# damesek/hnsw-clj

Hardware: AMD Instinct MI355X
Metric: QPS @ recall@10>=0.98 (31k x 768, k=10); IVF scan achieved HBM GB/s vs roofline (higher is better)
Workload: dtype f32; 1 GPU; hnsw search-knn (ultra_fast.clj:346-374 = graph.clj:297-320), 31,173 x 768 f32 (clustered, java.util.Random seed 42; queries: the same generator, seed 43), k=10, M=16 ef_construction=200, index built on the device by the heuristic builder, batched HIP traversal kernel; builder=heuristic, ef_search=640, parallelism=replicas x1 (index replicated, queries sharded, no collective)

## Files before the change

hnsw-clj_amd/csrc/dense.hip:

```cpp
#include "engine.hpp"
#include "dense_kernels.hpp"
#include "wave_kernels.hpp"

namespace hg {

template <int N, int R, bool L>
static HnswKernelFn wave_dense_kernel(const HnswLaunchPlan &p) {
    return p.vis_global ? &hnsw_wave_kernel<N, R, L, true, false, true> : &hnsw_wave_kernel<N, R, L, false, false, true>;
}

HnswKernelFn hnsw_wave_dense_kernel_for(const HnswLaunchPlan &p, const HnswArgs &a) {
    const bool l2 = a.metric == METRIC_L2;
    if (p.nch == 3 && p.dense_rows == 4) return l2 ? wave_dense_kernel<3, 4, true>(p) : wave_dense_kernel<3, 4, false>(p);
#define PICK(N, R, RF) return l2 ? wave_dense_kernel<N, RF, true>(p) : wave_dense_kernel<N, RF, false>(p)
    HG_HNSW_ROWS(p.nch, 2, PICK);
#undef PICK
}

size_t hnsw_dense_code_bytes(int nch, int32_t nq) {
    return (sizeof(uint32_t) * 2 * kWave * nch * static_cast<size_t>(nq) + 255) & ~static_cast<size_t>(255);
}

int64_t hnsw_dense_ld(int64_t n) { return (n + kDenseTR - 1) / kDenseTR * kDenseTR; }

int launch_hnsw_dense(const hnswgpu_index *idx, const float *d_Q, int64_t qld, int32_t nq, void *codes, float *lb, int64_t lb_ld,
                      hipStream_t st) {
    QueryCodeArgs c;
    c.Q = d_Q;
    c.qld = qld;
    c.dim = idx->dim;
    c.nq = nq;
    c.qcode = static_cast<uint32_t *>(codes);
    c.qscal = reinterpret_cast<QueryScal *>(static_cast<char *>(codes) + hnsw_dense_code_bytes(idx->nch, nq));
    const int blocks = (nq + kNWave - 1) / kNWave;
#define CALL(N, R, L) hipLaunchKernelGGL((hnsw_query_code_kernel<N>), dim3(blocks), dim3(kWG), 0, st, c)
    HG_DISPATCH(idx->nch, false, CALL);
#undef CALL
    HG_HIP(hipGetLastError());
    DenseArgs d;
    d.qcode = c.qcode;
    d.qscal = c.qscal;
    d.qrows = idx->d_qrows;
    d.qmeta = idx->d_qmeta;
    d.lb = lb;
    d.lb_ld = lb_ld;
    d.n = idx->n;
    d.nq = nq;
    d.kbytes = 4 * kWave * idx->nch;
    d.metric = idx->metric;
    d.nqt = (nq + kDenseTQ - 1) / kDenseTQ;
    d.nrt = static_cast<int32_t>((idx->n + kDenseTR - 1) / kDenseTR);
    d.rp = std::max(1, std::min(kDensePanel, d.nrt / 8));
    d.nsp = (d.nrt + d.rp - 1) / d.rp;
    const int64_t grid = 8LL * ((d.nsp + 7) / 8) * d.nqt * d.rp;
    HG_REQUIRE(grid < (1LL << 31), HNSWGPU_ELIMIT, "too many tiles for one bounds launch");
    hipLaunchKernelGGL(hnsw_dense_bounds_kernel, dim3(static_cast<unsigned>(grid)), dim3(kWG), 0, st, d);
    HG_HIP(hipGetLastError());
    return 0;
}

}
```

hnsw-clj_amd/csrc/dense_kernels.hpp:

```cpp
#pragma once
#include "kernels.hpp"

namespace hg {

typedef int dense_v4i __attribute__((ext_vector_type(4)));
typedef int dense_v16i __attribute__((ext_vector_type(16)));

constexpr int kDenseTQ = 128;
constexpr int kDenseTR = 128;
constexpr int kDenseKS = 128;
constexpr int kDensePanel = 8;

struct QueryCodeArgs {
    const float *Q;
    int64_t qld;
    int32_t dim;
    int32_t nq;
    uint32_t *qcode;
    QueryScal *qscal;
};

template <int NCH>
__global__ __launch_bounds__(kWG) void hnsw_query_code_kernel(QueryCodeArgs a) {
    const int lane = threadIdx.x & (kWave - 1);
    const int qi = blockIdx.x * kNWave + (threadIdx.x >> 6);
    if (qi >= a.nq) return;
    float4 q[NCH];
    load_query<NCH>(q, a.Q + static_cast<int64_t>(qi) * a.qld, a.dim, lane);
    Query16<NCH> qc;
    encode_query16<NCH>(q, qc);
    uint32_t *hi = a.qcode + (static_cast<int64_t>(2 * qi) * kWave + lane) * NCH, *lo = hi + kWave * NCH;
#pragma unroll
    for (int c = 0; c < NCH; c++) {
        hi[c] = qc.hi[c];
        lo[c] = qc.lo[c];
    }
    if (lane == 0) a.qscal[qi] = qc.sc;
}

struct DenseArgs {
    const uint32_t *qcode;
    const QueryScal *qscal;
    const uint32_t *qrows;
    const float4 *qmeta;
    float *lb;
    int64_t lb_ld;
    int64_t n;
    int32_t nq;
    int32_t kbytes;
    int32_t metric;
    int32_t nqt, nrt;
    int32_t rp;
    int32_t nsp;
};

__device__ __forceinline__ int dense_lds_off(int row, int ks) { return row * kDenseKS + ((ks ^ ((row >> 1) & 7)) << 4); }

__global__ __launch_bounds__(kWG, 2) void hnsw_dense_bounds_kernel(DenseArgs a) {
    __shared__ __align__(16) unsigned char s_a[2 * kDenseTQ * kDenseKS];
    __shared__ __align__(16) unsigned char s_b[kDenseTR * kDenseKS];
    __shared__ QueryScal s_scal[kDenseTQ];
    const int tid = threadIdx.x, lane = tid & (kWave - 1), wv = tid >> 6;
    const int l31 = lane & 31, half = lane >> 5;
    const int xcd = blockIdx.x & 7, j = blockIdx.x >> 3;
    const int per = a.nqt * a.rp;
    const int sp = (j / per) * 8 + xcd, rem = j % per;
    const int qt = rem / a.rp, rt = sp * a.rp + rem % a.rp;
    if (sp >= a.nsp || rt >= a.nrt) return;
    const int q0 = qt * kDenseTQ;
    const int64_t r0 = static_cast<int64_t>(rt) * kDenseTR;
    const int64_t K = a.kbytes;

    if (tid < kDenseTQ) s_scal[tid] = a.qscal[q0 + tid < a.nq ? q0 + tid : a.nq - 1];
    const int ks = tid & 7, rr = tid >> 3;
    const unsigned char *const pa = reinterpret_cast<const unsigned char *>(a.qcode) + ks * 16;
    const unsigned char *const pb = reinterpret_cast<const unsigned char *>(a.qrows) + ks * 16;
    const int64_t a_last = 2LL * a.nq - 1, b_last = a.n - 1;
    dense_v4i va[8], vb[4];
#define HG_DENSE_FETCH(k0)                                                                       \
    do {                                                                                         \
        _Pragma("unroll") for (int i = 0; i < 8; i++) {                                          \
            const int64_t ar = static_cast<int64_t>(2 * q0) + rr + 32 * i;                       \
            va[i] = *reinterpret_cast<const dense_v4i *>(pa + (ar < a_last ? ar : a_last) * K + (k0)); \
        }                                                                                        \
        _Pragma("unroll") for (int i = 0; i < 4; i++) {                                          \
            const int64_t br = r0 + rr + 32 * i;                                                 \
            vb[i] = *reinterpret_cast<const dense_v4i *>(pb + (br < b_last ? br : b_last) * K + (k0)); \
        }                                                                                        \
    } while (0)
    dense_v16i acc[4][2];
#pragma unroll
    for (int sa = 0; sa < 4; sa++)
#pragma unroll
        for (int sb = 0; sb < 2; sb++)
#pragma unroll
            for (int g = 0; g < 16; g++) acc[sa][sb][g] = 0;
    const int arow = (wv >> 1) * 128 + l31, brow = (wv & 1) * 64 + l31;
    HG_DENSE_FETCH(0);
    for (int k0 = 0; k0 < a.kbytes; k0 += kDenseKS) {
#pragma unroll
        for (int i = 0; i < 8; i++) *reinterpret_cast<dense_v4i *>(s_a + dense_lds_off(rr + 32 * i, ks)) = va[i];
#pragma unroll
        for (int i = 0; i < 4; i++) *reinterpret_cast<dense_v4i *>(s_b + dense_lds_off(rr + 32 * i, ks)) = vb[i];
        __syncthreads();
        if (k0 + kDenseKS < a.kbytes) HG_DENSE_FETCH(k0 + kDenseKS);
#pragma unroll
        for (int u = 0; u < kDenseKS / 32; u++) {
            dense_v4i fa[4], fb[2];
#pragma unroll
            for (int sb = 0; sb < 2; sb++) fb[sb] = *reinterpret_cast<const dense_v4i *>(s_b + dense_lds_off(brow + 32 * sb, 2 * u + half));
#pragma unroll
            for (int sa = 0; sa < 4; sa++) fa[sa] = *reinterpret_cast<const dense_v4i *>(s_a + dense_lds_off(arow + 32 * sa, 2 * u + half));
#pragma unroll
            for (int sa = 0; sa < 4; sa++)
#pragma unroll
                for (int sb = 0; sb < 2; sb++) acc[sa][sb] = __builtin_amdgcn_mfma_i32_32x32x32_i8(fa[sa], fb[sb], acc[sa][sb], 0, 0, 0);
        }
        __syncthreads();
    }
#undef HG_DENSE_FETCH
#pragma unroll
    for (int sb = 0; sb < 2; sb++) {
        const int64_t row = r0 + (wv & 1) * 64 + 32 * sb + l31;
        const float4 meta = a.qmeta[row < a.n ? row : a.n - 1];
#pragma unroll
        for (int sa = 0; sa < 4; sa++) {
#pragma unroll
            for (int g = 0; g < 8; g++) {
                const int ql = (wv >> 1) * 64 + 16 * sa + 4 * (g >> 1) + 2 * half + (g & 1);
                const int tot = static_cast<int>(static_cast<unsigned>(acc[sa][sb][2 * g]) * 256u + static_cast<unsigned>(acc[sa][sb][2 * g + 1]));
                const float lb = code_lower_bound(a.metric, tot, s_scal[ql], meta, meta.w);
                if (q0 + ql < a.nq && row < a.n) a.lb[static_cast<int64_t>(q0 + ql) * a.lb_ld + row] = lb;
            }
        }
    }
}

}
```

hnsw-clj_amd/csrc/hnsw.hip:

```cpp
#include <math.h>
#include <stdlib.h>
#include <string.h>

#include <algorithm>
#include <chrono>
#include <condition_variable>
#include <functional>
#include <mutex>
#include <thread>
#include <vector>

#include "build_kernels.hpp"
#include "engine.hpp"
#include "hnsw_remove_kernels.hpp"
#include "hnsw_update_kernels.hpp"
#include "ivf_update_ids.hpp"
#include "lsh_remove_ids.hpp"
#include "javarandom.hpp"
#include "order_kernels.hpp"
#include "parts_kernels.hpp"
#include "solo_kernels.hpp"

namespace hg {

constexpr size_t kMaxLds = 160 * 1024;

static size_t hnsw_lds_bytes(int cap, int nwords, int nw) {
    return sizeof(uint2) * cap + sizeof(int32_t) * 3 * kMaxDeg + sizeof(int32_t) * 16 + sizeof(int32_t) * nw * kWave +
           sizeof(uint2) * kPfRing + sizeof(uint32_t) * nwords + sizeof(uint16_t) * cap + 16;
}

static size_t wave_lds_bytes(int cap, int nwords) {
    return sizeof(uint2) * cap + sizeof(uint2) * kWave + 2 * sizeof(int32_t) * kMaxDeg + sizeof(uint32_t) * nwords + 16;
}

constexpr int64_t kLdsVisitedMaxRows = 262144;
static_assert(kLdsVisitedMaxRows <= (1 << 18), "solo_tag holds 18 bits of a node id");
static bool hnsw_vis_global(int64_t n, int64_t vis_global_env) { return vis_global_env != 0 || n > kLdsVisitedMaxRows; }

constexpr int kPfMaxQueries = 128;
static_assert(kPfMaxQueries == kSoloMaxQueries, "one bound for both kinds of small launch");
constexpr int kSoloMinEf = 96;
constexpr int kOrderMinQueries = 10000;

static void hnsw_calibration_absorb(hnswgpu_index *idx) {
    if (idx->hnsw_cal_state != 1 || !idx->ev_hnsw_cal || hipEventQuery(idx->ev_hnsw_cal) != hipSuccess) return;
    const double f32_rows = static_cast<double>(idx->hnsw_cal_host[0]), nb = static_cast<double>(idx->hnsw_cal_host[1]);
    idx->hnsw_cal_frac = nb > 0 ? f32_rows / nb : 0.0;
    const double keep = static_cast<double>(tune(HNSWGPU_TUNE_HNSW_CALIBRATE_PCT, 65)) / 100.0;
    idx->hnsw_rej_off = nb > 0 && idx->hnsw_cal_frac > keep;
    idx->hnsw_cal_state = 2;
}

template <int N, int R, bool L>
static HnswKernelFn search_kernel(const HnswLaunchPlan &p) {
    if (p.kernel == HnswKernel::SearchHelpers) return &hnsw_search_kernel<N, R, L, 4, false, true>;
    if (p.vis_global) return p.nw == 1 ? &hnsw_search_kernel<N, R, L, 1, true> : (p.nw == 2 ? &hnsw_search_kernel<N, R, L, 2, true> : &hnsw_search_kernel<N, R, L, 4, true>);
    return p.nw == 1 ? &hnsw_search_kernel<N, R, L, 1, false> : (p.nw == 2 ? &hnsw_search_kernel<N, R, L, 2, false> : &hnsw_search_kernel<N, R, L, 4, false>);
}

static HnswKernelFn hnsw_search_kernel_for(const HnswLaunchPlan &p, const HnswArgs &a) {
    const bool l2 = a.metric == METRIC_L2;
#define PICK(N, R, RF) HG_HNSW_ROWS_IN_FLIGHT(search_kernel, N, R, RF)
    HG_HNSW_ROWS(p.nch, 2, PICK);
#undef PICK
}

static int hnsw_launch_plan(const hnswgpu_index *idx, const HnswArgs &a, const HnswLaunchPlan *first, HnswLaunchPlan &p,
                            bool plain_search = false) {
    memset(&p, 0, sizeof(p));
    const bool build = a.q_rows != nullptr, repeat = a.q_index != nullptr;
    const bool parts = a.items != nullptr;
    const int64_t vis_rows = parts ? idx->max_part : a.n;
    p.nch = idx->nch;
    p.rejection = a.qrows && (idx->rejection_mode == 2 || (idx->rejection_mode == 1 && a.nq >= 2 * idx->cus && idx->dim >= 128));
    if (p.rejection && idx->rejection_mode == 1 && !build && !repeat && tune(HNSWGPU_TUNE_HNSW_CALIBRATE, 1) != 0) {
        if (idx->hnsw_cal_state == 2 && idx->hnsw_rej_off) p.rejection = false;
        p.calibrate = idx->hnsw_cal_state == 0 && !(idx->prof && idx->d_rej_stats);
    }
    if (repeat) {
        p.kernel = HnswKernel::Search;
        p.vis_global = first->vis_global;
        p.nw = 4;
        p.grid = std::min(a.nq, 256);
    } else {
        const int64_t nw_raw = tune(HNSWGPU_TUNE_HNSW_NW, 0);
        const int nw_env = (nw_raw == 1 || nw_raw == 2 || nw_raw == 4) ? static_cast<int>(nw_raw) : 0;
        p.vis_global = hnsw_vis_global(vis_rows, tune(HNSWGPU_TUNE_VIS_GLOBAL, 0));
        const int64_t pf_env = tune(HNSWGPU_TUNE_PREFETCH, kTuneUnset);
        const int helper_groups = pf_env == kTuneUnset ? 4 : static_cast<int>(std::max<int64_t>(0, std::min<int64_t>(16, pf_env)));
        const int solo_groups = pf_env == kTuneUnset ? 8 : static_cast<int>(std::max<int64_t>(0, std::min<int64_t>(31, pf_env)));
        const bool small = helper_groups > 0 && !p.vis_global && !build && !parts && a.nq <= kPfMaxQueries && nw_env == 0 &&
                           a.n < (1LL << 31) && a.M0 <= kMaxDeg;
        const int64_t solo_mode = tune(HNSWGPU_TUNE_SOLO, 1);
        const bool solo = small && solo_groups > 0 && (solo_mode >= 2 || (solo_mode == 1 && a.ef >= kSoloMinEf));
        const int64_t hints_env = tune(HNSWGPU_TUNE_PF_HINTS, kTuneUnset);
        const auto hints = [hints_env](int dflt) {
            return static_cast<int32_t>(std::max<int64_t>(1, std::min<int64_t>(32, hints_env == kTuneUnset ? dflt : hints_env)));
        };
        int nw = nw_env > 0 ? nw_env : (a.nq > 1536 ? 1 : (a.nq > 768 ? 2 : 4));
        if (nw_env == 0 && p.rejection && p.nch <= 3) nw = a.nq > 2048 ? 1 : (a.nq > 1024 ? 2 : 4);
        const int nwords = p.vis_global ? 0 : a.nwords;
        const int64_t wave_mode = tune(HNSWGPU_TUNE_HNSW_WAVE, 1);
        const bool wave = wave_mode != 0 && !small && nw_env == 0 && wave_lds_bytes(a.cap, nwords) <= kMaxLds && a.M0 <= kMaxDeg &&
                          (wave_mode >= 2 || nw == 1 || a.ef >= 640);
        if (nw_env == 0 && !wave)
            while (nw < 4 && static_cast<int64_t>(kMaxLds / hnsw_lds_bytes(a.cap, nwords, nw)) * nw < 13) nw *= 2;
        p.grid = a.nq;
        if (solo) {
            p.kernel = HnswKernel::Solo;
            p.rejection = false;
            p.pf_groups = std::max(1, std::min(solo_groups, idx->cus / std::max(a.nq, 1) - 1));
            p.pf_hints = hints(a.ef < 256 ? 8 : 16);
            p.solo_chase = tune(HNSWGPU_TUNE_SOLO_CHASE, 1) != 0 ? 1 : 0;
            p.grid = 8 * ((a.nq + 7) / 8) * (1 + p.pf_groups);
            int log2s = static_cast<int>(tune(HNSWGPU_TUNE_SOLO_SLOTS, 0));
            if (log2s <= 0) {
                const int64_t want = std::min<int64_t>(a.n, 32LL * a.ef);
                log2s = 11;
                while ((1LL << log2s) < want && log2s < 18) log2s++;
                while (log2s > 11 && (static_cast<int64_t>(a.nq) << log2s) * a.M0 * 8 > (512LL << 20)) log2s--;
            }
            p.solo_log2s = std::max(8, std::min(log2s, 18));
            const size_t S = static_cast<size_t>(1) << p.solo_log2s;
            p.mail_bytes = (sizeof(uint32_t) * kSoloMailWords * kSoloMaxQueries + 255) & ~static_cast<size_t>(255);
            p.table_bytes = (sizeof(uint32_t) * S * a.nq + 255) & ~static_cast<size_t>(255);
            p.rec_bytes = sizeof(unsigned long long) * S * a.M0 * a.nq;
        } else if (small) {
            p.kernel = HnswKernel::SearchHelpers;
            nw = 4;
            p.pf_groups = std::max(1, std::min(helper_groups, idx->cus / std::max(a.nq, 1) - 1));
            p.pf_hints = hints(4);
            p.grid = 8 * ((a.nq + 7) / 8) * (1 + p.pf_groups);
            p.mail_bytes = sizeof(uint32_t) * kPfMailWords * kPfMaxQueries;
            p.table_bytes = sizeof(unsigned long long) * kPfMaxQueries * kPfRing * kMaxDeg;
            p.pf_eval = tune(HNSWGPU_TUNE_PF_EVAL, 1) != 0;
            if (p.pf_eval) p.rejection = false;
        } else {
            p.kernel = wave ? HnswKernel::Wave : HnswKernel::Search;
        }
        p.region = p.mail_bytes + p.table_bytes + p.rec_bytes;
        p.nw = nw;
        const int64_t order_mode = tune(HNSWGPU_TUNE_HNSW_ORDER, 1);
        p.ordered = p.kernel == HnswKernel::Wave && !build && !parts && idx->d_qrows && idx->d_qmeta &&
                    (order_mode >= 2 || (order_mode == 1 && a.nq >= kOrderMinQueries));
        if (p.ordered) p.grid = 8 * ((a.nq + 7) / 8);
        p.lb_ld = hnsw_dense_ld(a.n);
        const bool dense_rule = a.nq >= 8 * idx->cus && 6.5 * a.ef >= 0.06 * static_cast<double>(a.n);
        p.dense = plain_search && p.kernel == HnswKernel::Wave && p.rejection && !build && !parts && idx->dense_mode != 0 &&
                  static_cast<double>(a.nq) * static_cast<double>(p.lb_ld) * sizeof(float) <= static_cast<double>(idx->dense_budget) &&
                  (idx->dense_mode >= 2 || dense_rule);
        constexpr size_t kDenseRows4Lds = 7680;
        if (p.dense && p.nch == 3)
            p.dense_rows = idx->dense_rows_mode != 0 ? idx->dense_rows_mode : (wave_lds_bytes(a.cap, nwords) > kDenseRows4Lds ? 4 : 2);
    }
    p.nwords = p.vis_global ? 0 : a.nwords;
    if (p.vis_global) {
        const int64_t budget = 16LL << 30;
        int64_t max_wg = budget / (4 * std::max<int64_t>(a.n, 1));
        max_wg = std::min<int64_t>(std::max<int64_t>(max_wg, 256), 256 * 12);
        const int64_t slots = p.ordered ? 8 * ((static_cast<int64_t>(a.nq) + 7) / 8) : a.nq;
        p.grid = static_cast<int>(std::min<int64_t>(slots, max_wg));
        if (p.ordered) p.grid = std::max(8, p.grid & ~7);
        p.gens = (slots + p.grid - 1) / p.grid * (a.max_level + 1);
    }
    p.block = p.kernel == HnswKernel::Solo ? kWG : (p.kernel == HnswKernel::Wave ? kWave : p.nw * kWave);
    p.lds = p.kernel == HnswKernel::Solo   ? solo_lds_bytes(a.cap, p.nwords)
            : p.kernel == HnswKernel::Wave ? wave_lds_bytes(a.cap, p.nwords)
                                           : hnsw_lds_bytes(a.cap, p.nwords, p.nw);
    HG_REQUIRE(p.lds <= kMaxLds, HNSWGPU_ELIMIT, "HNSW search state (%zu B: ef=%d, n=%lld) exceeds the 160 KiB LDS of a CU", p.lds,
               a.ef, (long long)a.n);
    p.calibrate = p.calibrate && p.rejection;
    if (!build && !repeat) {
        const size_t fixed = hnsw_lds_bytes(0, p.nwords, 4);
        const int64_t cap_max = std::min<int64_t>(65000, static_cast<int64_t>((kMaxLds - fixed) / (sizeof(uint2) + sizeof(uint16_t))));
        const int64_t big = std::min<int64_t>(cap_max - a.ef, vis_rows);
        p.repeat_cap = big > kGhost ? static_cast<int32_t>(a.ef + big) : 0;
    }
    p.fn = parts                          ? hnsw_parts_kernel_for(p, a)
           : p.kernel == HnswKernel::Solo ? hnsw_solo_kernel_for(p, a)
           : p.dense                      ? hnsw_wave_dense_kernel_for(p, a)
           : p.kernel == HnswKernel::Wave ? hnsw_wave_kernel_for(p, a)
                                          : hnsw_search_kernel_for(p, a);
    HG_REQUIRE(p.fn, HNSWGPU_ELIMIT, "unsupported row length");
    return 0;
}

static int hnsw_tables_idle(hnswgpu_index *idx, hipStream_t st) {
    for (auto &sl : idx->slots)
        if (sl.st) HG_HIP(hipStreamSynchronize(sl.st));
    if (idx->stream) HG_HIP(hipStreamSynchronize(idx->stream));
    HG_HIP(hipStreamSynchronize(st));
    return 0;
}

static int hnsw_number_launch(hnswgpu_index *idx, hipStream_t st) {
    idx->pf_seq = (idx->pf_seq + 1) & 0xffffff;
    if ((idx->pf_seq & 0x3fff) != 0) return 0;
    HG_TRY(hnsw_tables_idle(idx, st));
    for (DevBuf *t : {&idx->s_pf, &idx->s_solo})
        if (t->p) HG_HIP(hipMemsetAsync(t->p, 0, t->cap, st));
    HG_HIP(hipStreamSynchronize(st));
    idx->pf_seq++;
    return 0;
}

static int hnsw_launch_resources(hnswgpu_index *idx, const HnswLaunchPlan &p, HnswArgs &a, hipStream_t st, int32_t *order_mem,
                                 DenseScratch *dense_mem) {
    a.dbg = g_tile_dbg_buf;
    if (p.dense) {
        DenseScratch &ds = dense_mem ? *dense_mem : idx->s_dense;
        HG_TRY(ds.codes.ensure(hnsw_dense_code_bytes(p.nch, a.nq) + sizeof(QueryScal) * static_cast<size_t>(a.nq)));
        HG_TRY(ds.lb.ensure(sizeof(float) * static_cast<size_t>(a.nq) * static_cast<size_t>(p.lb_ld)));
        HG_TRY(launch_hnsw_dense(idx, a.Q, a.qld, a.nq, ds.codes.p, ds.lb.as<float>(), p.lb_ld, st));
        a.lb = ds.lb.as<float>();
        a.lb_ld = p.lb_ld;
        idx->dense_launches++;
        if (p.dense_rows == 4) idx->dense_rows4_launches++;
    }
    if (p.ordered) {
        if (!order_mem) {
            HG_TRY(idx->s_hord.ensure(sizeof(int32_t) * 2 * static_cast<size_t>(a.nq)));
            order_mem = idx->s_hord.as<int32_t>();
        }
        OrderArgs o;
        o.Q = a.Q;
        o.qld = a.qld;
        o.dim = a.dim;
        o.metric = a.metric;
        o.nq = a.nq;
        o.n = a.n;
        o.qrows = idx->d_qrows;
        o.qmeta = idx->d_qmeta;
        o.order = order_mem;
        o.keys = order_mem + a.nq;
        HG_TRY(launch_hnsw_order(p.nch, o, st));
        a.q_order = o.order;
        idx->hnsw_order_last = o.order;
        idx->hnsw_order_nq = a.nq;
    }
    a.rej_stats = idx->prof ? idx->d_rej_stats : nullptr;
    if (!p.rejection) a.qrows = nullptr;
    a.nwords = p.nwords;
    if (p.kernel == HnswKernel::SearchHelpers || p.kernel == HnswKernel::Solo) {
        const bool solo = p.kernel == HnswKernel::Solo;
        DevBuf &tab = solo ? idx->s_solo : idx->s_pf;
        if (tab.cap < 4 * p.region) {
            if (solo) HG_TRY(hnsw_tables_idle(idx, st));
            HG_TRY(tab.ensure(4 * p.region));
            HG_HIP(hipMemsetAsync(tab.p, 0, tab.cap, st));
            HG_HIP(hipStreamSynchronize(st));
        }
        HG_TRY(hnsw_number_launch(idx, st));
        a.pf_seq = idx->pf_seq;
        a.pf_groups = p.pf_groups;
        a.pf_hints = p.pf_hints;
        char *reg = static_cast<char *>(tab.p) + (idx->pf_seq & 3) * (solo ? (tab.cap / 4 & ~static_cast<size_t>(255)) : p.region);
        a.pf_mail = reinterpret_cast<uint32_t *>(reg);
        if (solo) {
            a.solo_chase = p.solo_chase;
            a.solo_log2s = p.solo_log2s;
            a.solo_claim = reinterpret_cast<uint32_t *>(reg + p.mail_bytes);
            a.solo_rec = reinterpret_cast<unsigned long long *>(reg + p.mail_bytes + p.table_bytes);
        } else if (p.pf_eval) {
            a.pf_res = reinterpret_cast<unsigned long long *>(reg + p.mail_bytes);
        }
    }
    if (p.vis_global) {
        const size_t need = sizeof(uint32_t) * static_cast<size_t>(a.n) * p.grid;
        if (need > idx->s_vis.cap) {
            HG_TRY(idx->s_vis.ensure(need));
            HG_HIP(hipMemsetAsync(idx->s_vis.p, 0, idx->s_vis.cap, st));
            idx->vis_gen = 0;
        }
        if (static_cast<int64_t>(idx->vis_gen) + p.gens >= 0xfffffff0LL) {
            HG_HIP(hipMemsetAsync(idx->s_vis.p, 0, idx->s_vis.cap, st));
            idx->vis_gen = 0;
        }
        a.vis = idx->s_vis.as<uint32_t>();
        a.vis_stride = a.n;
        a.gen_base = idx->vis_gen;
        idx->vis_gen += static_cast<uint32_t>(p.gens);
    }
    if (p.calibrate) {
        if (!idx->d_hnsw_cal) {
            HG_HIP(hipMalloc(reinterpret_cast<void **>(&idx->d_hnsw_cal), 2 * sizeof(unsigned long long)));
            HG_HIP(hipHostMalloc(reinterpret_cast<void **>(&idx->hnsw_cal_host), 2 * sizeof(unsigned long long), hipHostMallocDefault));
            HG_HIP(hipEventCreateWithFlags(&idx->ev_hnsw_cal, hipEventDisableTiming));
        }
        HG_HIP(hipMemsetAsync(idx->d_hnsw_cal, 0, 2 * sizeof(unsigned long long), st));
        a.rej_stats = idx->d_hnsw_cal;
    }
    return 0;
}

static int hnsw_dispatch(const HnswLaunchPlan &p, const HnswArgs &a, hipStream_t st) {
    if (p.lds > 48 * 1024)
        HG_HIP(hipFuncSetAttribute(reinterpret_cast<const void *>(p.fn), hipFuncAttributeMaxDynamicSharedMemorySize, static_cast<int>(p.lds)));
    hipLaunchKernelGGL(p.fn, dim3(p.grid), dim3(p.block), p.lds, st, a);
    HG_HIP(hipGetLastError());
    return 0;
}

static int hnsw_launch_planned(hnswgpu_index *idx, const HnswLaunchPlan &p, HnswArgs a, hipStream_t st, int32_t *order_mem = nullptr,
                               DenseScratch *dense_mem = nullptr) {
    HG_TRY(hnsw_launch_resources(idx, p, a, st, order_mem, dense_mem));
    HG_TRY(hnsw_dispatch(p, a, st));
    if (p.kernel == HnswKernel::Solo) count_launch(HNSWGPU_COUNT_HNSW_SOLO);
    else if (p.kernel == HnswKernel::SearchHelpers) count_launch(HNSWGPU_COUNT_HNSW_HELPERS);
    else count_launch(p.rejection ? HNSWGPU_COUNT_HNSW_REJECTION : HNSWGPU_COUNT_HNSW_PLAIN);
    if (p.kernel == HnswKernel::Wave) count_launch(HNSWGPU_COUNT_HNSW_WAVE);
    if (p.ordered) count_launch(HNSWGPU_COUNT_HNSW_ORDERED);
    if (p.calibrate) {
        HG_HIP(hipMemcpyAsync(idx->hnsw_cal_host, idx->d_hnsw_cal, 2 * sizeof(unsigned long long), hipMemcpyDeviceToHost, st));
        HG_HIP(hipEventRecord(idx->ev_hnsw_cal, st));
        idx->hnsw_cal_state = 1;
    }
    return 0;
}

static int launch_hnsw_idx(hnswgpu_index *idx, const HnswArgs &a, hipStream_t st) {
    if (a.nq <= 0) return 0;
    HnswLaunchPlan p;
    hnsw_calibration_absorb(idx);
    HG_TRY(hnsw_launch_plan(idx, a, nullptr, p));
    return hnsw_launch_planned(idx, p, a, st);
}

static void free_graph(hnswgpu_index *idx) {
    idx->graph_gen++;
    idx->build_flags = 0;
    idx->hnsw_cal_state = 0;
    idx->hnsw_rej_off = false;
    void *ptrs[] = {idx->d_levels, idx->d_l0, idx->d_upadj, idx->d_upoff};
    for (void *p : ptrs)
        if (p) (void)hipFree(p);
    idx->d_levels = idx->d_l0 = idx->d_upadj = nullptr;
    idx->d_upoff = nullptr;
    idx->has_graph = false;
    if (idx->d_parts) (void)hipFree(idx->d_parts);
    idx->d_parts = nullptr;
    idx->nparts = 0;
    idx->max_part = 0;
    idx->h_part_off.clear();
    idx->h_part_entry.clear();
    idx->h_part_level.clear();
}

static int alloc_graph(hnswgpu_index *idx, int M, int M0, int64_t up_blocks) {
    int64_t n = std::max<int64_t>(idx->n, 1);
    HG_HIP(hipMalloc(reinterpret_cast<void **>(&idx->d_levels), sizeof(int32_t) * n));
    HG_HIP(hipMalloc(reinterpret_cast<void **>(&idx->d_l0), sizeof(int32_t) * n * M0));
    HG_HIP(hipMalloc(reinterpret_cast<void **>(&idx->d_upoff), sizeof(int64_t) * (n + 1)));
    HG_HIP(hipMalloc(reinterpret_cast<void **>(&idx->d_upadj), sizeof(int32_t) * std::max<int64_t>(up_blocks, 1) * M));
    idx->M = M;
    idx->M0 = M0;
    idx->up_blocks = up_blocks;
    return 0;
}

static void fill_args(const hnswgpu_index *idx, HnswArgs &a) {
    memset(&a, 0, sizeof(a));
    a.rows = idx->d_base;
    a.row_norms = idx->d_norms;
    a.qrows = idx->d_qrows;
    a.qmeta = idx->d_qmeta;
    a.ld = idx->ld;
    a.n = idx->n;
    a.dim = idx->dim;
    a.metric = idx->metric;
    a.l0_adj = idx->d_l0;
    a.M0 = idx->M0;
    a.up_off = idx->d_upoff;
    a.up_adj = idx->d_upadj;
    a.M = idx->M;
    a.entry = idx->entry;
    a.max_level = idx->max_level;
    a.nwords = static_cast<int32_t>((idx->n + 31) / 32);
}

struct SlotSignal {
    int32_t *again;
    uint32_t *done_cnt;
    uint32_t *host_flag;
    int32_t *host_again;
    uint32_t flag_val;
    int32_t *order;
    DenseScratch *dense;
};

static int search_enqueue(hnswgpu_index *idx, const float *d_Q, int32_t nq, int32_t k, int32_t ef,
                          int32_t *d_ids, float *d_dist, int64_t *d_stats, hipStream_t st,
                          const SlotSignal *sig = nullptr, bool repeat_only = false, bool filtered = false) {
    HG_REQUIRE(idx->nparts == 0, HNSWGPU_ESTATE,
               "the index holds a forest (hnswgpu_set_graph_parts / hnswgpu_hnsw_build_parts): search it with hnswgpu_hnsw_search_parts");
    HnswArgs a;
    fill_args(idx, a);
    a.Q = d_Q;
    a.qld = idx->dim;
    a.nq = nq;
    a.ef = ef;
    a.k = k;
    a.cap = ef + kGhost;
    a.out_ids = d_ids;
    a.out_dist = d_dist;
    a.stats = d_stats;
    if (nq <= 0) return 0;
    HnswLaunchPlan p;
    if (!repeat_only) hnsw_calibration_absorb(idx);
    HG_TRY(hnsw_launch_plan(idx, a, nullptr, p, !filtered));
    int32_t *again_cnt, *again;
    if (sig) {
        again_cnt = sig->again;
        again = again_cnt + 1;
    } else {
        HG_TRY(idx->s_probes.ensure(sizeof(int32_t) * (static_cast<size_t>(nq) + 1)));
        again_cnt = idx->s_probes.as<int32_t>();
        again = again_cnt + 1;
        HG_HIP(hipMemsetAsync(again_cnt, 0, sizeof(int32_t), st));
    }
    int rc = 0;
    if (!repeat_only) {
        a.again = again;
        a.again_cnt = again_cnt;
        if (sig) {
            a.done_cnt = sig->done_cnt;
            a.host_flag = sig->host_flag;
            a.host_again = sig->host_again;
            a.flag_val = sig->flag_val;
        }
        hipEvent_t e0;
        prof_begin(idx, PROF_HNSW, st, &e0);
        rc = hnsw_launch_planned(idx, p, a, st, sig ? sig->order : nullptr, sig ? sig->dense : nullptr);
        prof_end(idx, PROF_HNSW, st, e0);
        if (rc || sig) return rc;
        a.done_cnt = nullptr;
        a.host_flag = nullptr;
    }
    if (p.repeat_cap) {
        a.cap = p.repeat_cap;
        a.again = nullptr;
        a.again_cnt = nullptr;
        a.q_index = again;
        a.nq_dev = again_cnt;
        HnswLaunchPlan r;
        HG_TRY(hnsw_launch_plan(idx, a, &p, r));
        rc = hnsw_launch_planned(idx, r, a, st);
    }
    if (repeat_only && rc == 0) HG_HIP(hipMemsetAsync(again_cnt, 0, sizeof(int32_t), st));
    return rc;
}
// ... 2113 lines not shown
```

Measured before the change: 1.035 million queries/s.

## Make dense bounds kernel persistent with double-buffered LDS and larger row tiles

Rewrites the int8 MFMA lower-bound kernel as a persistent kernel that walks tiles with a CU-sized grid. It uses 512-thread workgroups, 256-row tiles and double-buffered dynamic LDS, and prefetches the next tile's codes, scales and metadata while the current tile's MFMAs run. The metric becomes a template parameter and full tiles skip bounds checks on stores. It also lowers the ef/n threshold for choosing the dense path. Costs are heavier LDS and register use, lower occupancy, and load imbalance from the static tile stride.

```diff
diff --git a/hnsw-clj_amd/csrc/dense.hip b/hnsw-clj_amd/csrc/dense.hip
--- a/hnsw-clj_amd/csrc/dense.hip
+++ b/hnsw-clj_amd/csrc/dense.hip
@@ -21,7 +21,7 @@
     return (sizeof(uint32_t) * 2 * kWave * nch * static_cast<size_t>(nq) + 255) & ~static_cast<size_t>(255);
 }
 
-int64_t hnsw_dense_ld(int64_t n) { return (n + kDenseTR - 1) / kDenseTR * kDenseTR; }
+int64_t hnsw_dense_ld(int64_t n) { return (n + kDenseLd - 1) / kDenseLd * kDenseLd; }
 
 int launch_hnsw_dense(const hnswgpu_index *idx, const float *d_Q, int64_t qld, int32_t nq, void *codes, float *lb, int64_t lb_ld,
                       hipStream_t st) {
@@ -47,14 +47,26 @@
     d.n = idx->n;
     d.nq = nq;
     d.kbytes = 4 * kWave * idx->nch;
-    d.metric = idx->metric;
-    d.nqt = (nq + kDenseTQ - 1) / kDenseTQ;
-    d.nrt = static_cast<int32_t>((idx->n + kDenseTR - 1) / kDenseTR);
-    d.rp = std::max(1, std::min(kDensePanel, d.nrt / 8));
-    d.nsp = (d.nrt + d.rp - 1) / d.rp;
-    const int64_t grid = 8LL * ((d.nsp + 7) / 8) * d.nqt * d.rp;
-    HG_REQUIRE(grid < (1LL << 31), HNSWGPU_ELIMIT, "too many tiles for one bounds launch");
-    hipLaunchKernelGGL(hnsw_dense_bounds_kernel, dim3(static_cast<unsigned>(grid)), dim3(kWG), 0, st, d);
+    dense_tiling(d);
+    const int64_t places = dense_walk_places(d);
+    const unsigned grid = static_cast<unsigned>(std::min<int64_t>(places, std::max(8, idx->cus / 8 * 8)));
+    HG_REQUIRE(places < (1LL << 31) - grid, HNSWGPU_ELIMIT, "too many tiles for one bounds launch");
+    d.nvt = static_cast<int32_t>(places);
+    static bool attr_done[3][64] = {};
+#define CALL(M)                                                                                                              \
+    do {                                                                                                                     \
+        if (attr_needed(attr_done[M]))                                                                                       \
+            HG_HIP(hipFuncSetAttribute(reinterpret_cast<const void *>(&hnsw_dense_bounds_kernel<M>),                         \
+                                       hipFuncAttributeMaxDynamicSharedMemorySize, kDenseLds));                              \
+        hipLaunchKernelGGL((hnsw_dense_bounds_kernel<M>), dim3(grid), dim3(kDenseWG), kDenseLds, st, d);                     \
+    } while (0)
+    static_assert(METRIC_COS == 0 && METRIC_L2 == 1 && METRIC_DOT == 2, "attr_done");
+    switch (idx->metric) {
+        case METRIC_L2: CALL(METRIC_L2); break;
+        case METRIC_DOT: CALL(METRIC_DOT); break;
+        default: CALL(METRIC_COS); break;
+    }
+#undef CALL
     HG_HIP(hipGetLastError());
     return 0;
 }
diff --git a/hnsw-clj_amd/csrc/dense_kernels.hpp b/hnsw-clj_amd/csrc/dense_kernels.hpp
--- a/hnsw-clj_amd/csrc/dense_kernels.hpp
+++ b/hnsw-clj_amd/csrc/dense_kernels.hpp
@@ -7,9 +7,13 @@
 typedef int dense_v16i __attribute__((ext_vector_type(16)));
 
 constexpr int kDenseTQ = 128;
-constexpr int kDenseTR = 128;
+constexpr int kDenseTR = 256;
+constexpr int kDenseLd = 128;
 constexpr int kDenseKS = 128;
-constexpr int kDensePanel = 8;
+constexpr int kDensePanel = 4;
+constexpr int kDenseWG = 512;
+constexpr int kDenseImage = (2 * kDenseTQ + kDenseTR) * kDenseKS;
+constexpr int kDenseLds = 2 * kDenseImage + 2 * (kDenseTQ * 32 + kDenseTR * 16);
 
 struct QueryCodeArgs {
     const float *Q;
@@ -48,92 +52,177 @@
     int64_t n;
     int32_t nq;
     int32_t kbytes;
-    int32_t metric;
     int32_t nqt, nrt;
     int32_t rp;
     int32_t nsp;
+    int32_t nvt;
 };
 
+inline void dense_tiling(DenseArgs &d) {
+    d.nqt = (d.nq + kDenseTQ - 1) / kDenseTQ;
+    d.nrt = static_cast<int32_t>((d.n + kDenseTR - 1) / kDenseTR);
+    d.rp = d.nrt / 8 < 1 ? 1 : d.nrt / 8 < kDensePanel ? d.nrt / 8 : kDensePanel;
+    d.nsp = (d.nrt + d.rp - 1) / d.rp;
+}
+inline int64_t dense_walk_places(const DenseArgs &d) { return 8LL * ((d.nsp + 7) / 8) * d.nqt * d.rp; }
+
 __device__ __forceinline__ int dense_lds_off(int row, int ks) { return row * kDenseKS + ((ks ^ ((row >> 1) & 7)) << 4); }
 
-__global__ __launch_bounds__(kWG, 2) void hnsw_dense_bounds_kernel(DenseArgs a) {
-    __shared__ __align__(16) unsigned char s_a[2 * kDenseTQ * kDenseKS];
-    __shared__ __align__(16) unsigned char s_b[kDenseTR * kDenseKS];
-    __shared__ QueryScal s_scal[kDenseTQ];
-    const int tid = threadIdx.x, lane = tid & (kWave - 1), wv = tid >> 6;
-    const int l31 = lane & 31, half = lane >> 5;
-    const int xcd = blockIdx.x & 7, j = blockIdx.x >> 3;
-    const int per = a.nqt * a.rp;
+__device__ __forceinline__ bool dense_tile_at(const DenseArgs &a, int v, int &qt, int &rt) {
+    const int xcd = v & 7, j = v >> 3, per = a.nqt * a.rp;
     const int sp = (j / per) * 8 + xcd, rem = j % per;
-    const int qt = rem / a.rp, rt = sp * a.rp + rem % a.rp;
-    if (sp >= a.nsp || rt >= a.nrt) return;
-    const int q0 = qt * kDenseTQ;
-    const int64_t r0 = static_cast<int64_t>(rt) * kDenseTR;
-    const int64_t K = a.kbytes;
-
-    if (tid < kDenseTQ) s_scal[tid] = a.qscal[q0 + tid < a.nq ? q0 + tid : a.nq - 1];
-    const int ks = tid & 7, rr = tid >> 3;
-    const unsigned char *const pa = reinterpret_cast<const unsigned char *>(a.qcode) + ks * 16;
-    const unsigned char *const pb = reinterpret_cast<const unsigned char *>(a.qrows) + ks * 16;
-    const int64_t a_last = 2LL * a.nq - 1, b_last = a.n - 1;
-    dense_v4i va[8], vb[4];
-#define HG_DENSE_FETCH(k0)                                                                       \
-    do {                                                                                         \
-        _Pragma("unroll") for (int i = 0; i < 8; i++) {                                          \
-            const int64_t ar = static_cast<int64_t>(2 * q0) + rr + 32 * i;                       \
-            va[i] = *reinterpret_cast<const dense_v4i *>(pa + (ar < a_last ? ar : a_last) * K + (k0)); \
-        }                                                                                        \
-        _Pragma("unroll") for (int i = 0; i < 4; i++) {                                          \
-            const int64_t br = r0 + rr + 32 * i;                                                 \
-            vb[i] = *reinterpret_cast<const dense_v4i *>(pb + (br < b_last ? br : b_last) * K + (k0)); \
-        }                                                                                        \
-    } while (0)
-    dense_v16i acc[4][2];
-#pragma unroll
-    for (int sa = 0; sa < 4; sa++)
-#pragma unroll
-        for (int sb = 0; sb < 2; sb++)
-#pragma unroll
-            for (int g = 0; g < 16; g++) acc[sa][sb][g] = 0;
-    const int arow = (wv >> 1) * 128 + l31, brow = (wv & 1) * 64 + l31;
-    HG_DENSE_FETCH(0);
-    for (int k0 = 0; k0 < a.kbytes; k0 += kDenseKS) {
-#pragma unroll
-        for (int i = 0; i < 8; i++) *reinterpret_cast<dense_v4i *>(s_a + dense_lds_off(rr + 32 * i, ks)) = va[i];
-#pragma unroll
-        for (int i = 0; i < 4; i++) *reinterpret_cast<dense_v4i *>(s_b + dense_lds_off(rr + 32 * i, ks)) = vb[i];
-        __syncthreads();
-        if (k0 + kDenseKS < a.kbytes) HG_DENSE_FETCH(k0 + kDenseKS);
-#pragma unroll
-        for (int u = 0; u < kDenseKS / 32; u++) {
-            dense_v4i fa[4], fb[2];
-#pragma unroll
-            for (int sb = 0; sb < 2; sb++) fb[sb] = *reinterpret_cast<const dense_v4i *>(s_b + dense_lds_off(brow + 32 * sb, 2 * u + half));
-#pragma unroll
-            for (int sa = 0; sa < 4; sa++) fa[sa] = *reinterpret_cast<const dense_v4i *>(s_a + dense_lds_off(arow + 32 * sa, 2 * u + half));
-#pragma unroll
-            for (int sa = 0; sa < 4; sa++)
-#pragma unroll
-                for (int sb = 0; sb < 2; sb++) acc[sa][sb] = __builtin_amdgcn_mfma_i32_32x32x32_i8(fa[sa], fb[sb], acc[sa][sb], 0, 0, 0);
-        }
-        __syncthreads();
-    }
-#undef HG_DENSE_FETCH
-#pragma unroll
-    for (int sb = 0; sb < 2; sb++) {
-        const int64_t row = r0 + (wv & 1) * 64 + 32 * sb + l31;
-        const float4 meta = a.qmeta[row < a.n ? row : a.n - 1];
-#pragma unroll
-        for (int sa = 0; sa < 4; sa++) {
-#pragma unroll
-            for (int g = 0; g < 8; g++) {
-                const int ql = (wv >> 1) * 64 + 16 * sa + 4 * (g >> 1) + 2 * half + (g & 1);
+    qt = rem / a.rp;
+    rt = sp * a.rp + rem % a.rp;
+    return sp < a.nsp && rt < a.nrt;
+}
+
+template <int METRIC, bool FULL>
+__device__ __forceinline__ void dense_store_bounds(const dense_v16i (&acc)[4][2], const QueryScal *sc, const float4 (&meta)[2],
+                                                   float *out, int64_t lb_ld, int nql, const bool (&row_ok)[2]) {
+#pragma unroll
+    for (int sa = 0; sa < 4; sa++) {
+#pragma unroll
+        for (int g = 0; g < 8; g++) {
+            const int c = 16 * sa + 4 * (g >> 1) + (g & 1);
+            const QueryScal q = sc[c];
+#pragma unroll
+            for (int sb = 0; sb < 2; sb++) {
                 const int tot = static_cast<int>(static_cast<unsigned>(acc[sa][sb][2 * g]) * 256u + static_cast<unsigned>(acc[sa][sb][2 * g + 1]));
-                const float lb = code_lower_bound(a.metric, tot, s_scal[ql], meta, meta.w);
-                if (q0 + ql < a.nq && row < a.n) a.lb[static_cast<int64_t>(q0 + ql) * a.lb_ld + row] = lb;
+                const float lb = code_lower_bound(METRIC, tot, q, meta[sb], meta[sb].w);
+                if (FULL || (c < nql && row_ok[sb])) out[c * lb_ld + 32 * sb] = lb;
             }
         }
     }
 }
 
-}
+template <int METRIC>
+__global__ __launch_bounds__(kDenseWG, 2) void hnsw_dense_bounds_kernel(DenseArgs a) {
+    static_assert(sizeof(QueryScal) == 32 && sizeof(float4) == 16, "kDenseLds");
+    extern __shared__ __align__(16) unsigned char smem[];
+    QueryScal *const s_scal = reinterpret_cast<QueryScal *>(smem + 2 * kDenseImage);
+    float4 *const s_meta = reinterpret_cast<float4 *>(smem + 2 * kDenseImage + 2 * kDenseTQ * 32);
+    const int tid = threadIdx.x, lane = tid & (kWave - 1), wv = __builtin_amdgcn_readfirstlane(tid >> 6);
+    const int l31 = lane & 31, half = lane >> 5;
+    const int64_t K = a.kbytes;
+    const int nk = a.kbytes / kDenseKS;
+    const int step = gridDim.x;
+    int v = blockIdx.x, qt = 0, rt = 0;
+    while (v < a.nvt && !dense_tile_at(a, v, qt, rt)) v += step;
+    if (v >= a.nvt) return;
+
+    const int ks = tid & 7, rr = tid >> 3;
+    const int64_t a_last = 2LL * a.nq - 1, b_last = a.n - 1;
+    const unsigned char *pa[4], *pb[4];
+    dense_v4i va[4], vb[4], vs;
+    float4 vm;
+    int q0, par = 0;
+    int64_t r0;
+#define HG_DENSE_TILE()                                                                                               \
+    do {                                                                                                              \
+        q0 = qt * kDenseTQ;                                                                                           \
+        r0 = static_cast<int64_t>(rt) * kDenseTR;                                                                     \
+        _Pragma("unroll") for (int i = 0; i < 4; i++) {                                                               \
+            const int64_t ar = 2LL * q0 + rr + 64 * i, br = r0 + rr + 64 * i;                                         \
+            pa[i] = reinterpret_cast<const unsigned char *>(a.qcode) + (ar < a_last ? ar : a_last) * K + ks * 16;     \
+            pb[i] = reinterpret_cast<const unsigned char *>(a.qrows) + (br < b_last ? br : b_last) * K + ks * 16;     \
+        }                                                                                                             \
+        const int tq = q0 + ((tid >> 1) & (kDenseTQ - 1));                                                            \
+        const int64_t tr = r0 + (tid & (kDenseTR - 1));                                                               \
+        vs = reinterpret_cast<const dense_v4i *>(a.qscal + (tq < a.nq ? tq : a.nq - 1))[tid & 1];                     \
+        vm = a.qmeta[tr < a.n ? tr : a.n - 1];                                                                        \
+    } while (0)
+#define HG_DENSE_TERMS(p)                                                                                             \
+    do {                                                                                                              \
+        if (tid < 2 * kDenseTQ) reinterpret_cast<dense_v4i *>(s_scal + (p) * kDenseTQ)[tid] = vs;                     \
+        if (tid < kDenseTR) s_meta[(p) * kDenseTR + tid] = vm;                                                        \
+    } while (0)
+#define HG_DENSE_FETCH(k0)                                                                               \
+    do {                                                                                                 \
+        _Pragma("unroll") for (int i = 0; i < 4; i++) va[i] = *reinterpret_cast<const dense_v4i *>(pa[i] + (k0)); \
+        _Pragma("unroll") for (int i = 0; i < 4; i++) vb[i] = *reinterpret_cast<const dense_v4i *>(pb[i] + (k0)); \
+    } while (0)
+#define HG_DENSE_WRITE(im)                                                                                            \
+    do {                                                                                                              \
+        _Pragma("unroll") for (int i = 0; i < 4; i++)                                                                 \
+            *reinterpret_cast<dense_v4i *>(smem + (im) * kDenseImage + dense_lds_off(rr + 64 * i, ks)) = va[i];       \
+        _Pragma("unroll") for (int i = 0; i < 4; i++)                                                                 \
+            *reinterpret_cast<dense_v4i *>(smem + (im) * kDenseImage + 2 * kDenseTQ * kDenseKS + dense_lds_off(rr + 64 * i, ks)) = vb[i]; \
+    } while (0)
+#define HG_DENSE_MUL(im)                                                                                              \
+    do {                                                                                                              \
+        const unsigned char *const s_a = smem + (im) * kDenseImage, *const s_b = s_a + 2 * kDenseTQ * kDenseKS;       \
+        _Pragma("unroll") for (int u = 0; u < kDenseKS / 32; u++) {                                                   \
+            dense_v4i fa[4], fb[2];                                                                                   \
+            _Pragma("unroll") for (int sb = 0; sb < 2; sb++)                                                          \
+                fb[sb] = *reinterpret_cast<const dense_v4i *>(s_b + dense_lds_off(brow + 32 * sb, 2 * u + half));     \
+            _Pragma("unroll") for (int sa = 0; sa < 4; sa++)                                                          \
+                fa[sa] = *reinterpret_cast<const dense_v4i *>(s_a + dense_lds_off(arow + 32 * sa, 2 * u + half));     \
+            _Pragma("unroll") for (int sa = 0; sa < 4; sa++)                                                          \
+                _Pragma("unroll") for (int sb = 0; sb < 2; sb++)                                                      \
+                    acc[sa][sb] = __builtin_amdgcn_mfma_i32_32x32x32_i8(fa[sa], fb[sb], acc[sa][sb], 0, 0, 0);        \
+        }                                                                                                             \
+    } while (0)
+
+    const int arow = (wv >> 2) * 128 + l31, brow = (wv & 3) * 64 + l31;
+    HG_DENSE_TILE();
+    HG_DENSE_FETCH(0);
+    HG_DENSE_TERMS(0);
+    HG_DENSE_WRITE(0);
+    HG_DENSE_FETCH(kDenseKS);
+    __syncthreads();
+    for (;;) {
+        dense_v16i acc[4][2];
+#pragma unroll
+        for (int sa = 0; sa < 4; sa++)
+#pragma unroll
+            for (int sb = 0; sb < 2; sb++)
+#pragma unroll
+                for (int g = 0; g < 16; g++) acc[sa][sb][g] = 0;
+        const int eq0 = q0, epar = par;
+        const int64_t er0 = r0;
+        bool more = false;
+        for (int s = 0; s < nk; s += 2) {
+            const bool last = s + 2 >= nk;
+            HG_DENSE_MUL(0);
+            HG_DENSE_WRITE(1);
+            if (!last) {
+                HG_DENSE_FETCH((s + 2) * kDenseKS);
+            } else {
+                v += step;
+                while (v < a.nvt && !dense_tile_at(a, v, qt, rt)) v += step;
+                more = v < a.nvt;
+                if (more) {
+                    par ^= 1;
+                    HG_DENSE_TILE();
+                    HG_DENSE_FETCH(0);
+                }
+            }
+            __syncthreads();
+            HG_DENSE_MUL(1);
+            if (!last || more) {
+                if (last) HG_DENSE_TERMS(par);
+                HG_DENSE_WRITE(0);
+                HG_DENSE_FETCH(last ? kDenseKS : (s + 3) * kDenseKS);
+            }
+            __syncthreads();
+        }
+        const int cq = eq0 + (wv >> 2) * 64 + 2 * half;
+        const int64_t crow = er0 + (wv & 3) * 64 + l31;
+        const bool full = eq0 + kDenseTQ <= a.nq && er0 + kDenseTR <= a.n;
+        const QueryScal *const sc = s_scal + epar * kDenseTQ + (wv >> 2) * 64 + 2 * half;
+        const float4 *const sm = s_meta + epar * kDenseTR + (wv & 3) * 64 + l31;
+        const float4 meta[2] = {sm[0], sm[32]};
+        const bool row_ok[2] = {crow < a.n, crow + 32 < a.n};
+        float *const out = a.lb + static_cast<int64_t>(cq) * a.lb_ld + crow;
+        if (full) dense_store_bounds<METRIC, true>(acc, sc, meta, out, a.lb_ld, 0, row_ok);
+        else dense_store_bounds<METRIC, false>(acc, sc, meta, out, a.lb_ld, a.nq - cq, row_ok);
+        if (!more) break;
+    }
+#undef HG_DENSE_MUL
+#undef HG_DENSE_WRITE
+#undef HG_DENSE_FETCH
+#undef HG_DENSE_TERMS
+#undef HG_DENSE_TILE
+}
+
+}
diff --git a/hnsw-clj_amd/csrc/hnsw.hip b/hnsw-clj_amd/csrc/hnsw.hip
--- a/hnsw-clj_amd/csrc/hnsw.hip
+++ b/hnsw-clj_amd/csrc/hnsw.hip
@@ -146,7 +146,7 @@
                     (order_mode >= 2 || (order_mode == 1 && a.nq >= kOrderMinQueries));
         if (p.ordered) p.grid = 8 * ((a.nq + 7) / 8);
         p.lb_ld = hnsw_dense_ld(a.n);
-        const bool dense_rule = a.nq >= 8 * idx->cus && 6.5 * a.ef >= 0.06 * static_cast<double>(a.n);
+        const bool dense_rule = a.nq >= 8 * idx->cus && 6.5 * a.ef >= 0.02 * static_cast<double>(a.n);
         p.dense = plain_search && p.kernel == HnswKernel::Wave && p.rejection && !build && !parts && idx->dense_mode != 0 &&
                   static_cast<double>(a.nq) * static_cast<double>(p.lb_ld) * sizeof(float) <= static_cast<double>(idx->dense_budget) &&
                   (idx->dense_mode >= 2 || dense_rule);
```

After: 1.069 million queries/s, median of 6. 3.4% higher.
